# ilirlikalla/Smith-Waterman-FPGA-module

Hardware: AMD Instinct MI355X
Metric: GCUPS (higher is better)
Workload: dtype f16

## Files before the change

### smith-waterman-fpga-module_amd/csrc/swbank_bank.h

```cpp
#ifndef SWBANK_BANK_H
#define SWBANK_BANK_H

#include <dlfcn.h>
#include <hip/hip_runtime.h>
#include <rccl/rccl.h>

#include <algorithm>
#include <cmath>
#include <cstdarg>
#include <cstdio>
#include <cstdlib>
#include <cstring>
#include <atomic>
#include <condition_variable>
#include <functional>
#include <memory>
#include <mutex>
#include <numeric>
#include <thread>
#include <chrono>
#include <vector>
#if defined(__SSE2__)
#include <emmintrin.h>
#endif
// ... 341 lines not shown

 private:
  void loop(int device) {
    (void)hipSetDevice(device);
    for (;;) {
      std::function<sw_status()> f;
      {
        std::unique_lock<std::mutex> l(m_);
        cv_.wait(l, [&] { return stop_ || !q_.empty(); });
        if (q_.empty()) return;
        f = std::move(q_.front());
        q_.erase(q_.begin());
      }
      if (st_.load(std::memory_order_relaxed) == SW_OK) {
        const sw_status s = f();
        if (s != SW_OK) st_.store(s, std::memory_order_release);
      }
      done_.fetch_add(1, std::memory_order_acq_rel);
    }
  }
  std::mutex m_;
  std::condition_variable cv_;
  std::vector<std::function<sw_status()>> q_;
  bool stop_ = false;
  size_t posted_ = 0;
  std::atomic<size_t> done_{0};
  std::atomic<sw_status> st_{SW_OK};
  std::thread th_;
};

struct sw_bank {
  sw_config cfg{};
  int device = 0;
  int cus = 0;
  hipStream_t stream = nullptr;
  char err[512] = {0};

  bool have_pen = false;
  int alpha = SW_DNA_ALPHA;
  std::vector<int8_t> matrix;
  int32_t gap_open = 0, gap_extend = 0;

  bool have_query = false;
  uint64_t qid = 0;
  std::vector<uint8_t> query;
  std::vector<std::vector<uint8_t>> qset;
  bool mq_ready = false;
  DevBuf<uint32_t> mqtab, mqtab16;
  size_t mq_words = 0;
  DevBuf<uint32_t> mqpair;
  size_t mq_pair_words = 0;
  int mq_pair_segs = 0, mq_pair_rows = 0;
  uint32_t mq_pS1 = 0, mq_pS2 = 0;

  bool dirty = true;
  int R = 32, RB = 4, W = 1, col0 = 0, prof = 0;
  uint32_t S = 0, O = 0, E = 0, nv = 0, PS = 0, pad = 4;
  int32_t smax = 0;
  DevBuf<uint32_t> qtab;
  bool f16 = false;
  uint32_t nv16 = 0, PS16 = 0;
  int32_t f16_neg = 0;
  DevBuf<uint32_t> qtab16;
  DevBuf<uint32_t> qpair;
  uint32_t pair_bytes = 0, pS1 = 0, pS2 = 0;
  DevBuf<uint32_t> qpair_skew, skew_ctab;
  uint32_t skew_entries = 0;
  int32_t skew_neg = 0;
  DevBuf<uint32_t> fb_idx, fb_cnt;
  bool i32_ready = false;
  uint32_t i32_strips = 0;
  DevBuf<uint2> i32prof, i32scr;
  DevBuf<unsigned long long> best_key;
  bool al_ready = false;
  DevBuf<uint8_t> al_tab, al_res, al_hs;
  DevBuf<uint2> al_scr;
  DevBuf<uint32_t> al_dirs, al_lens, al_cig, al_list, al_hq;
  DevBuf<uint64_t> al_offs;
  DevBuf<sw_alignment> al_out;
  DevBuf<SwkAlignPlan> al_plan;
  DevBuf<unsigned long long> top_state, top_keys;
  DevBuf<int32_t> top_scores, top_hsc;
  DevBuf<uint64_t> top_hits;
  DevBuf<uint32_t> top_cnt;
  hipEvent_t ev_top = nullptr;
  SliceScratch stat_slice;
  StagedBatch stat_host;
  DevBuf<unsigned long long> stat_cnt;
  DevBuf<double> stat_par;
  std::vector<double> stat_hpar;
  hipEvent_t ev_stat = nullptr;
  SliceScratch str_slice;
  StagedBatch str_host;
  DevBuf<uint8_t> str_hstr;
  DevBuf<int32_t> str_hsc;
  hipEvent_t ev_strand = nullptr;
  SliceScratch fr_slice, fr_hits;
  StagedBatch fr_host;
  DevBuf<uint32_t> fr_lens, fr_hit_lens, fr_hit_q;
  DevBuf<uint8_t> fr_hfr;
  DevBuf<int32_t> fr_hsc;
  hipEvent_t ev_frame = nullptr;
  using Seg = qtab::Seg;
  std::vector<Seg> segs;
  qtab::Plan plan;
  DevBuf<uint2> edge[2];
// ... 330 lines not shown
```

### smith-waterman-fpga-module_amd/csrc/swbank_bank.hip

```cpp
#include "swbank_bank.h"

sw_status fail(sw_bank* b, sw_status st, const char* fmt, ...) {
  if (b) {
    va_list ap;
    va_start(ap, fmt);
    vsnprintf(b->err, sizeof(b->err), fmt, ap);
    va_end(ap);
  }
  return st;
}

extern "C" int32_t sw_device_count(void) {
  int n = 0;
  if (hipGetDeviceCount(&n) != hipSuccess) return 0;
  return n;
}

static sw_status check_device(int dev) {
  int ndev = 0;
  if (hipGetDeviceCount(&ndev) != hipSuccess || ndev <= 0) return SW_ERR_NO_DEVICE;
  if (dev < 0 || dev >= ndev) return SW_ERR_NO_DEVICE;
  hipDeviceProp_t prop;
  if (hipGetDeviceProperties(&prop, dev) != hipSuccess) return SW_ERR_NO_DEVICE;
  if (std::strncmp(prop.gcnArchName, "gfx950", 6) != 0) return SW_ERR_NO_DEVICE;
// ... 495 lines not shown
  for (const auto& u : tables) words += u.second->size();
  TableUpload up(b);
  SWOK(up.begin(words * 4));
  for (const auto& u : tables) SWOK(up.put(*u.first, *u.second));
  SWOK(up.end());
  b->plan = p;
  b->segs = t.segs;
  b->R = p.R;
  b->RB = p.RB;
  b->W = t.segs[0].W;
  b->col0 = p.col0;
  b->prof = p.prof;
  b->S = (uint32_t)p.S;
  b->O = (uint32_t)p.o;
  b->E = (uint32_t)p.e;
  b->smax = p.smax;
  b->nv = p.nv;
  b->PS = p.PS;
  b->pad = p.pad;
  b->f16 = p.f16;
  b->nv16 = p.nv16;
  b->PS16 = p.PS16;
  b->f16_neg = p.f16_neg;
  b->pair_bytes = t.pair_words * 4;
  b->pS1 = t.pS1;
  b->pS2 = t.pS2;
  b->skew_entries = (uint32_t)t.tfloor.size();
  b->skew_neg = t.skew_neg;
  b->wK = p.wK;
  b->wsegs = p.wsegs;
  b->wPS = p.prof ? (uint32_t)(64 * p.wK) : 0;
  b->wPS16 = p.prof ? (uint32_t)(128 * p.wK) : 0;
  b->wseg_words = t.wt.size() / p.wsegs;
  b->wseg_words16 = t.wt16.size() / p.wsegs;
  for (int i = 0; i < 3; ++i) {
    b->sK[i] = p.sK[i];
    b->sseg_words[i] = t.st[i].size() / (2 << i);
    b->sseg_words16[i] = t.st16[i].size() / (2 << i);
    b->sPS[i] = p.prof ? (uint32_t)(64 * p.sK[i]) : 0;
    b->sPS16[i] = p.prof ? (uint32_t)(128 * p.sK[i]) : 0;
  }
  b->i32_ready = false;
  b->al_ready = false;
  b->mq_ready = false;
  b->dirty = false;
  return SW_OK;
}

sw_status prepare_multi(sw_bank* b) {
  if (b->mq_ready) return SW_OK;
  const qtab::SetTables t =
      qtab::build_set(b->plan, b->segs, b->matrix.data(), b->qset, table_options());
  TableUpload up(b);
  SWOK(up.begin((t.t8.size() + t.t16.size() + t.tp.size()) * 4));
  SWOK(up.put(b->mqtab, t.t8));
  SWOK(up.put(b->mqtab16, t.t16));
  SWOK(up.put(b->mqpair, t.tp));
  SWOK(up.end());
  b->mq_words = t.words;
  b->mq_pair_words = t.pair_words;
  b->mq_pair_segs = t.pair_segs;
  b->mq_pair_rows = t.pair_rows;
  b->mq_pS1 = t.pS1;
  b->mq_pS2 = t.pS2;
  b->mq_ready = true;
  return SW_OK;
}

sw_status prepare_i32(sw_bank* b) {
  if (b->i32_ready) return SW_OK;
  if (b->pad + 1 > 25)
    return fail(b, SW_ERR_UNSUPPORTED, "int32 kernel: alphabet %d too large", b->alpha);
  uint32_t strips = 0;
  const std::vector<int16_t> h =
      qtab::build_i32(b->matrix.data(), b->alpha, (int)b->S, b->pad, b->query.data(),
                      (uint32_t)b->query.size(), strips);
  TableUpload up(b);
  SWOK(up.begin(h.size() * 2));
  SWOK(up.put(b->i32prof, h));
  SWOK(up.end());
  b->i32_strips = strips;
  b->i32_ready = true;
  return SW_OK;
}

extern "C" sw_status sw_bank_set_timing(sw_bank* b, int32_t enable) {
  DevGuard dev_guard(b);
  if (!b) return SW_ERR_ARG;
  if (b->is_multi()) return each_kid(b, [&](sw_bank* k) { return sw_bank_set_timing(k, enable); });
  b->timing = enable != 0;
  return SW_OK;
}

extern "C" sw_status sw_bank_timing(sw_bank* b, uint64_t* launches, double* pack_ms,
                                    double* score_ms) {
  DevGuard dev_guard(b);
  if (!b) return SW_ERR_ARG;
  double p = 0, s = 0;
  uint64_t n = 0;
  sw_status st = SW_OK;
  if (b->is_multi()) {
    for (sw_bank* k : b->kids) {
      uint64_t kn = 0;
      double kp = 0, ks = 0;
      if ((st = sw_bank_timing(k, &kn, &kp, &ks)) != SW_OK)
        return fail(b, st, "device %d: %s", k->device, k->err);
      n += kn;
      p += kp;
      s += ks;
    }
    if (launches) *launches = n;
// ... 59 lines not shown
```

### smith-waterman-fpga-module_amd/csrc/swbank_ktile.hip

```cpp
#include "swbank_kcommon.h"

namespace swk {

template <int C>
__device__ __forceinline__ void tile_chunks_local(const Lane2& t, size_t tlo, size_t thi, size_t n,
                                                  int lane, int& nch, int& nfull, int& ncl,
                                                  int tile, uint32_t ulen) {
  if (ulen) {
    const bool any = (size_t)tile * SWB_TILE < n;
    const int lx = any ? (int)ulen : 0;
    nch = max(1, (lx + C - 1) / C);
    ncl = lx == 0 ? C : lx - C * (nch - 1);
    nfull = lx / C;
    return;
  }
  uint32_t Lmax = max(t.llo, t.lhi);
  uint32_t Lmin = min(tlo < n ? t.llo : ~0u, thi < n ? t.lhi : ~0u);
  uint32_t ol = (uint32_t)lane;
  asm volatile("" : "+v"(ol));
#pragma unroll
  for (int off = 32; off >= 1; off >>= 1) {
    const int ad = (int)((ol ^ (uint32_t)off) << 2);
    Lmax = max(Lmax, (uint32_t)__builtin_amdgcn_ds_bpermute(ad, (int)Lmax));
    Lmin = min(Lmin, (uint32_t)__builtin_amdgcn_ds_bpermute(ad, (int)Lmin));
  }
  const int lx = (int)__builtin_amdgcn_readfirstlane(Lmax);
  nch = max(1, (lx + C - 1) / C);
  ncl = lx == 0 ? C : lx - C * (nch - 1);
  const uint32_t lm = __builtin_amdgcn_readfirstlane(Lmin);
  nfull = lm == ~0u ? 0 : (int)(lm / C);
}

template <int R, int RB, bool COL0, bool PROF, bool GOTOH, bool F16, bool PAIR = false,
          bool MQ = false, bool STREAM = false, int C = 8, bool BAL = false, bool TRIM = false,
          bool SKEW = false, int NB = SKEW ? (TRIM ? SWK_SKEW_ACC_TRIM : SWK_SKEW_ACC) : 1>
__global__ void __launch_bounds__(R >= 64 ? 512 : 1024) score_kernel(const ScoreArgs a) {
  static_assert(!BAL || (!MQ && !STREAM && !COL0), "balanced ranges: one query, resident batch");
  static_assert(!TRIM || (BAL && PAIR), "trimmed last chunks: the balanced pair kernel");
  static_assert(!SKEW || (PAIR && F16 && !GOTOH && !MQ && !STREAM && R == 32 && C == 8),
                "SKEW: the merged f16 pair rows, one query, resident batch");
  static_assert(!MQ || !PROF, "several queries: row-LUT or pair-table variants");
  static_assert(!STREAM || (!MQ && !PROF), "streamed batches: single-query LUT / pair variants");
  static_assert(C == 8 || (C == 4 && PAIR && !STREAM), "4-column chunks: pair tables only");
  static_assert(!PAIR || ((R == 32 || (R == 16 && GOTOH)) && F16 && !PROF && !COL0 &&
                          (!GOTOH || !MQ)),
                "PAIR: f16, merged R = 32 or Gotoh R = 16 / 32 (one query)");
  extern __shared__ __attribute__((aligned(16))) uint32_t smem[];
  const int lane = threadIdx.x & 63;
  const int wave = __builtin_amdgcn_readfirstlane(threadIdx.x >> 6);
  const int W = __builtin_amdgcn_readfirstlane(blockDim.x >> 6);
  const bool seg_in = a.edge_in != nullptr, seg_out = a.edge_out != nullptr;
  uint32_t* bestsh = smem + (PAIR ? a.PS / 4 : 0);
  constexpr int RS = SWK_RING_ROW;
  uint2* ein = reinterpret_cast<uint2*>(bestsh + W * SWB_TILE);
  uint2* ring = ein + (seg_in ? 2 * C * RS : 0);
  uint8_t* prof = reinterpret_cast<uint8_t*>(ring + (size_t)(W > 1 ? 2 * (W - 1) : 1) * C * RS);

  size_t n = a.n;
  const uint32_t* idx = a.idx;
  if (idx && a.ident && __builtin_amdgcn_readfirstlane(*a.ident)) idx = nullptr;
  const uint32_t* sidx = TRIM ? a.sidx : nullptr;
  if (TRIM && sidx && a.ident && __builtin_amdgcn_readfirstlane(*a.ident)) sidx = nullptr;
  if (idx) {
    const uint32_t cnt = __builtin_amdgcn_readfirstlane(*a.nidx);
    n = cnt > a.idx_base ? min(a.n, (size_t)(cnt - a.idx_base)) : 0;
  }
  const int ntiles = (int)((n + SWB_TILE - 1) / SWB_TILE);
  const int G = (int)gridDim.x;
  const int nunits = MQ ? ntiles * (int)a.nq : ntiles;
  int total = 0;
  uint32_t packed = a.packed;
  int* sq = reinterpret_cast<int*>(prof);
  int bs = 0, bo = 0, be = 0, bf = 0;
  if constexpr (BAL && SKEW) {
    typedef __attribute__((address_space(4))) const uint32_t plan_u32;
    plan_u32* const pp = reinterpret_cast<plan_u32*>(reinterpret_cast<uintptr_t>(a.bal_plan)) +
                         (size_t)blockIdx.x * 4;
    bs = (int)pp[0], bo = (int)pp[1];
    be = (int)pp[4], bf = (int)pp[5];
    total = (int)(pp[6] - pp[2]);
  } else if constexpr (BAL) {
    const uint4 p0 = a.bal_plan[blockIdx.x], p1 = a.bal_plan[blockIdx.x + 1];
    bs = (int)__builtin_amdgcn_readfirstlane(p0.x), bo = (int)__builtin_amdgcn_readfirstlane(p0.y);
    be = (int)__builtin_amdgcn_readfirstlane(p1.x), bf = (int)__builtin_amdgcn_readfirstlane(p1.y);
    total = (int)__builtin_amdgcn_readfirstlane(p1.z - p0.z);
  }
  const auto bal_visit = [&](int v, int& t, int& c0, int& c1) {
    const int bK = -1;
    const int bfirst = bo ? bs + 1 : bs;
    const int hh = bf > 0 ? 1 : 0;
    if (v < hh) {
      t = be, c0 = 0, c1 = bf;
    } else if (v - hh < be - bfirst) {
// ... 328 lines not shown
        }
      }
      int ntile = nunit, nqq = q;
      if constexpr (MQ) {
        if (nunit < nunits) {
          if constexpr (PAIR) {
            ntile = nunit / (int)a.nq;
          } else {
            ntile = tile + G;
            while (ntile >= ntiles) {
              ntile -= ntiles;
              ++nqq;
            }
          }
        }
      }
      if (!last) {
        load_raw<C, !MQ>(cur, c + 1, c + 1 < nfull, a.pad, packed, rlo, rhi);
      } else if (nunit < nunits) {
        if constexpr (STREAM) cur = stream_tile(ntile, packed_n);
        else
          cur = lane_targets<!MQ>(a.res, a.offs, a.lens, n, ntile, lane, packed, idx, a.ulen,
                                  a.ustride);
        if constexpr (SKEW)
          tile_chunks_local<C>(cur, (size_t)ntile * SWB_TILE + lane,
                               (size_t)ntile * SWB_TILE + lane + 64, n, lane, nch_n, nfull_n, ncl_n,
                               ntile, TRIM ? 0u : a.ulen);
        else
          tile_chunks<C>(cur, (size_t)ntile * SWB_TILE + lane,
                         (size_t)ntile * SWB_TILE + lane + 64, n, nch_n, nfull_n, ncl_n);
        if (BAL && nvend >= 0 && nvend < nch_n) ncl_n = C;
        if (BAL && nvend < 0) nvend = nch_n;
        load_raw<C, !MQ>(cur, nc0, nc0 < nfull_n, a.pad, STREAM ? packed_n : packed, rlo, rhi);
      }
      const int slot = g & 1;
      if (seg_in && wave == 0 && (last ? nunit < nunits : (MQ ? unit : tile) < nunits))
        dma_edge_chunk<C>(a.edge_in + ((size_t)(last ? nunit : MQ ? unit : tile) * a.ecols +
                                    (size_t)(last ? 0 : c + 1) * C) * 64,
                       ein + (size_t)((g + 1) & 1) * C * RS, lane);
      int rl = lane;
      if constexpr (SKEW) asm volatile("" : "+v"(rl));
      uint2* rin = wave > 0 ? ring + ((size_t)((wave - 1) * 2 + slot) * C) * RS + rl
                   : seg_in ? ein + (size_t)slot * C * RS + rl
                            : ring + 64;
      uint2* rout = wave < W - 1 ? ring + ((size_t)(wave * 2 + slot) * C) * RS + rl
                    : W > 1      ? rin
                                 : ring + rl;
      const int cu = __builtin_amdgcn_readfirstlane(c);
      uint32_t cs[SKEW ? 7 + C : 1];
      if constexpr (SKEW) {
        cst_u32* const sl = ct + (cu * C + 2);
#pragma unroll
        for (int s = 0; s < 7 + C; ++s) cs[s] = sl[s];
        if (wave == 0 && lane == 0) {
#pragma unroll
          for (int jj = 0; jj < C; ++jj) {
            if constexpr (TRIM)
              ring[jj * RS + 64] = make_uint2(cs[jj + 7], SKEW_NEG);
            else
              __atomic_store_n(reinterpret_cast<__attribute__((address_space(3))) uint32_t*>(
                                   (size_t)(lds_void_ptr)&ring[jj * RS + 64].x),
                               cs[jj + 7], __ATOMIC_RELAXED);
          }
        }
      }
      (void)cu; (void)cs;
      uint2 rv = rin[0];
      ProfLookup16<PROF && F16 ? R : 2> lkq;
      (void)lkq;
      const int ncols = TRIM && c + 1 == nch ? ncl : C;
      bool trimmed = false;
      (void)ncols;
#pragma unroll
      for (int jj = 0; jj < C; ++jj) {
        if (TRIM && jj > 0 && __builtin_expect(jj >= ncols, 0)) {
          trimmed = true;
          break;
        }
        const u16x2 upH = as_u16x2(rv.x);
        u16x2 upX = as_u16x2(rv.y);
        if (jj + 1 < C) rv = rin[(jj + 1) * RS];
        u16x2 diag = prevUpH;
        prevUpH = upH;
        const uint32_t wlo = jj < 4 ? clo.x : clo.y, whi = jj < 4 ? chi.x : chi.y;
        if constexpr (PROF && F16) {
          const auto load16 = [&](int j, ProfLookup16<R>& out) {
            const uint32_t wl = j < 4 ? clo.x : clo.y, wh = j < 4 ? chi.x : chi.y;
            const uint32_t blo = min((wl >> (8 * (j & 3))) & 0xFFu, padc);
            const uint32_t bhi = min((wh >> (8 * (j & 3))) & 0xFFu, padc);
            const uint4* plo = reinterpret_cast<const uint4*>(prof + __umul24(blo, a.PS) + 2 * pbase);
            const uint4* phi = reinterpret_cast<const uint4*>(prof + __umul24(bhi, a.PS) + 2 * pbase);
#pragma unroll
            for (int q = 0; q < R / 8; ++q) {
              const uint4 x = plo[q], y = phi[q];
              out.lo[4 * q] = x.x; out.lo[4 * q + 1] = x.y; out.lo[4 * q + 2] = x.z;
              out.lo[4 * q + 3] = x.w;
              out.hi[4 * q] = y.x; out.hi[4 * q + 1] = y.y; out.hi[4 * q + 2] = y.z;
              out.hi[4 * q + 3] = y.w;
            }
          };
          ProfLookup16<R> lk;
          if (jj == 0) load16(0, lk);
          else lk = lkq;
          if (jj + 1 < C) load16(jj + 1, lkq);
          __builtin_amdgcn_sched_barrier(0);
          if (COL0 && jj == 0 && c == 0)
            column_f16<R, RB, GOTOH, true>(lk, diag, upX, Hl, Xl, best, NOE2, NE2, NO2);
// ... 373 lines not shown
  a.ctab = tab;
  a.f16_e1 = f16_pair((int)a.E);
  a.f16_ne8 = f16_pair(-8 * (int)a.E);
}

}

#define SWK_VARIANTS(X)                                                                       \
  X(16, 4, 0, 0, 0, 0) X(16, 4, 1, 0, 0, 0) X(32, 4, 0, 0, 0, 0) X(32, 4, 1, 0, 0, 0)         \
  X(32, 8, 0, 0, 0, 0) X(64, 4, 0, 0, 0, 0) X(64, 4, 1, 0, 0, 0)                              \
  X(16, 4, 0, 0, 1, 0) X(32, 4, 0, 0, 1, 0) X(64, 4, 0, 0, 1, 0)                              \
  X(16, 4, 0, 1, 0, 0) X(16, 4, 1, 1, 0, 0) X(32, 4, 0, 1, 0, 0) X(32, 4, 1, 1, 0, 0)         \
  X(64, 4, 0, 1, 0, 0) X(64, 4, 1, 1, 0, 0)                                                   \
  X(16, 4, 0, 1, 1, 0) X(32, 4, 0, 1, 1, 0) X(64, 4, 0, 1, 1, 0)                              \
  X(16, 4, 0, 0, 0, 1) X(16, 4, 1, 0, 0, 1) X(32, 4, 0, 0, 0, 1) X(64, 4, 0, 0, 0, 1)         \
  X(16, 4, 0, 0, 1, 1)                                                                        \
  X(16, 4, 0, 1, 0, 1) X(16, 4, 1, 1, 0, 1) X(16, 4, 0, 1, 1, 1) X(32, 4, 0, 0, 1, 1)


extern "C" int swk_has_variant(int R, int RB, int col0, int prof, int gotoh, int f16) {
#define SWK_HAS(RR, BB, C0, PF, GT, FH) \
  if (R == RR && RB == BB && col0 == C0 && prof == PF && gotoh == GT && f16 == FH) return 1;
  SWK_VARIANTS(SWK_HAS)
#undef SWK_HAS
  return 0;
}

extern "C" hipError_t swk_launch_score(int R, int RB, int col0, int prof, int gotoh, int f16,
                                       const uint8_t* res, const uint64_t* offs,
                                       const uint32_t* lens, size_t n, const uint32_t* qtab,
                                       uint32_t nv, uint32_t S, uint32_t O, uint32_t E,
                                       uint32_t PS, uint32_t pad, int W, int32_t* scores,
                                       const void* edge_in, void* edge_out, uint32_t ecols,
                                       int accum, int packed, const uint32_t* idx,
                                       const uint32_t* nidx, uint32_t idx_base,
                                       const uint32_t* ident, int pair, uint32_t pS1,
                                       uint32_t pS2, uint32_t ulen, uint32_t ustride,
                                       uint32_t nq, uint32_t qwords, size_t sstride,
                                       hipStream_t st, const uint32_t* skew_tab) {
  if (n == 0) return hipSuccess;
  swk::ScoreArgs a{res,  offs, lens, n,  qtab, nv, S,
                   O,    E,    PS,   pad, scores, static_cast<const uint2*>(edge_in),
                   static_cast<uint2*>(edge_out), ecols, (uint32_t)accum, (uint32_t)packed,
                   idx, nidx, idx_base, ident, pS1, pS2,
                   swk::f16_pair(-(int)(O + E)), swk::f16_pair(-(int)E),
                   swk::f16_pair(-(int)O), nullptr, 0u, 0u, 0};
  a.ulen = ulen;
  a.ustride = ustride;
  a.nq = nq;
  a.qwords = qwords;
  a.sstride = sstride;
  const uint32_t prof_bytes = (pad + 1) * PS;
  if (nq > 1 && pair) {
    if (R == 32 && f16 && !prof && !gotoh && !col0 && (W > 4 || a.edge_in || a.edge_out))
      return swk::launch_score<32, 4, false, false, false, true, true, true, false, 4>(a, W, 0, st);
    if (R == 32 && f16 && !prof && !gotoh && !col0)
      return swk::launch_score<32, 4, false, false, false, true, true, true>(a, W, 0, st);
    return hipErrorInvalidValue;
  }
  if (nq > 1) {
#define SWK_MQ_CASE(RR, GT, FH)                                                                  \
  if (R == RR && RB == 4 && !col0 && !prof && !pair && gotoh == GT && f16 == FH)                 \
    return swk::launch_score<RR, 4, false, false, (GT != 0), (FH != 0), false, true>(a, W, 0, st);
    SWK_MQ_CASE(32, 0, 1) SWK_MQ_CASE(32, 0, 0) SWK_MQ_CASE(16, 0, 1) SWK_MQ_CASE(16, 0, 0)
    SWK_MQ_CASE(16, 1, 1) SWK_MQ_CASE(16, 1, 0) SWK_MQ_CASE(32, 1, 1) SWK_MQ_CASE(32, 1, 0)
#undef SWK_MQ_CASE
    return hipErrorInvalidValue;
  }
  if (pair) {
    if (skew_tab && (R != 32 || !f16 || prof || gotoh || col0 || edge_in || edge_out || W > 4))
      return hipErrorInvalidValue;
    if (skew_tab) {
      swk::skew_args(a, skew_tab);
      return swk::launch_score<32, 4, false, false, false, true, true, false, false, 8, false,
                               false, true>(a, W, 0, st);
    }
    if (R == 32 && f16 && !prof && !gotoh && !col0)
      return swk::launch_score<32, 4, false, false, false, true, true>(a, W, 0, st);
#define SWK_GPAIR(RR)                                                                         \
    if (R == RR && f16 && !prof && gotoh && !col0) {                                          \
      const hipError_t e = a.edge_in || a.edge_out                                            \
          ? hipErrorInvalidConfiguration                                                      \
          : swk::launch_score<RR, 4, false, false, true, true, true>(a, W, 0, st);            \
      if (e != hipErrorInvalidConfiguration) return e;                                        \
      return swk::launch_score<RR, 4, false, false, true, true, true, false, false, 4>(a, W, 0, \
                                                                                         st); \
    }
    SWK_GPAIR(32) SWK_GPAIR(16)
#undef SWK_GPAIR
    return hipErrorInvalidValue;
  }
#define SWK_CASE(RR, BB, C0, PF, GT, FH)                                                      \
  if (R == RR && RB == BB && col0 == C0 && prof == PF && gotoh == GT && f16 == FH)            \
    return swk::launch_score<RR, BB, (C0 != 0), (PF != 0), (GT != 0), (FH != 0)>(a, W,        \
                                                                               prof_bytes, st);
  SWK_VARIANTS(SWK_CASE)
#undef SWK_CASE
  return hipErrorInvalidValue;
}

#if SWK_STAMPS
extern "C" void swk_set_stamps(void* p) { swk::g_stamps_host = static_cast<uint64_t*>(p); }
#endif

namespace swk {
__global__ void __launch_bounds__(256) bal_plan_uniform(uint4* plan, uint32_t ntiles, uint32_t K,
// ... 125 lines not shown
```

### smith-waterman-fpga-module_amd/csrc/swbank_launch.hip

```cpp
#include "swbank_bank.h"

static bool one_len_bin(uint32_t min_len, uint32_t max_len) {
  if (min_len > max_len) return false;
  uint32_t shift = 0;
  while ((max_len >> shift) >= 2048u) ++shift;
  return ((max_len - min_len) >> shift) == 0;
}

void u16_gotoh_rows(const sw_bank* b, bool f16, int& R, int& W) {
  if (f16 || !b->gotoh() || b->prof || R != 32 || b->segs.size() != 1 || b->query.size() > 256)
    return;
  R = 16;
  W = std::max(1, (int)((b->query.size() + 15) / 16));
}

bool wave_preferred(const sw_bank* b, size_t n, uint32_t max_len, bool use_f16) {
  const size_t nseg = b->segs.size();
  const size_t ntiles = (n + SWB_TILE - 1) / SWB_TILE;
  const bool gotoh = b->cfg.gap_model == SW_GAP_GOTOH;
  const double tiles = (double)ntiles, W = b->segs[0].W;
  const double cu_frac = std::min(1.0, tiles / 256.0);
  const double wps = std::min(4.0, std::max(1.0, std::ceil(tiles / 256.0)) * W / 4.0);
  const bool pair_tab = use_f16 && b->pair_bytes != 0 && env_int("SWBANK_PAIR", 1) != 0;
  const double tile_base = use_f16 ? (gotoh ? (b->prof ? 7100 : pair_tab ? 8500 : 7500)
// ... 401 lines not shown

sw_status track_best_device(sw_bank* b, const int32_t* d_scores, const uint64_t* d_ids, size_t n,
                            hipStream_t st) {
  if (n > 0xFFFFFFFFull) return SW_OK;
  HIPOK(b, b->best_key.reserve(1));
  HIPOK(b, b->best_dev.reserve(3));
  HIPOK(b, swk_best_hit(d_scores, d_ids, n, b->best_key.p, b->best_dev.p, b->best_dev.p + 2, st));
  if (!b->best_ev) HIPOK(b, hipEventCreateWithFlags(&b->best_ev, hipEventDisableTiming));
  HIPOK(b, hipEventRecord(b->best_ev, st));
  b->best_kind = 2;
  return SW_OK;
}

sw_status launch_set(sw_bank* b, const uint8_t* d_res, const uint64_t* d_offs,
                     const uint32_t* d_lens, size_t n, uint32_t min_len, uint32_t max_len,
                     int32_t* d_scores, hipStream_t st, size_t sstride) {
  const size_t nq = b->qset.size();
  const uint64_t smax = (uint64_t)std::max(0, b->smax);
  const uint64_t top = std::min<uint64_t>(b->query.size(), max_len) * smax + smax;
  const bool f16_ok = b->f16 && b->f16_neg >= -2048 && env_int("SWBANK_F16", 1) != 0;
  const bool use_f16 = f16_ok && top <= 2048u;
  const bool exact = use_f16 || top <= 65535u;
  const size_t ntiles = (n + SWB_TILE - 1) / SWB_TILE;
  const char* kforce = std::getenv("SWBANK_KERNEL");
  const bool mq = env_int("SWBANK_MQ", 1) != 0 && !b->prof && !b->col0 && exact &&
                  env_int("SWBANK_I32", 0) == 0 && (b->R == 16 || b->R == 32) && b->RB == 4 &&
                  n <= 0xFFFFFFFFull &&
                  !(kforce && std::strcmp(kforce, "wave") == 0) && ntiles * nq <= 0x7FFFFFFFull;
  if (!mq) {
    const std::vector<uint8_t> longest = b->query;
    sw_status rs = SW_OK;
    for (size_t i = 0; i < nq && rs == SW_OK; ++i) {
      b->query = b->qset[i];
      b->dirty = true;
      rs = prepare(b);
      if (rs == SW_OK)
        rs = launch(b, d_res, d_offs, d_lens, n, max_len, d_scores + i * sstride, st, SWK_PACK_BYTES,
                    nullptr, nullptr, true, true, nullptr, nullptr, 0, 0, min_len);
    }
    b->query = longest;
    b->dirty = true;
    const size_t L = strlen(b->last_kernel);
    snprintf(b->last_kernel + L, sizeof(b->last_kernel) - L, " x%zu queries", nq);
    return rs;
  }
  sw_status rs = prepare_multi(b);
  if (rs != SW_OK) return rs;
  const bool gotoh = b->gotoh();
  const int prow = std::max(b->mq_pair_rows, 32);
  const size_t slots = (prow > 256 ? 1 : prow > 128 ? 2 : 4) * (size_t)std::max(b->cus, 1);
  const bool mpair = b->mq_pair_segs > 0 && use_f16 && nq <= slots &&
                     8 * (slots - slots / nq * nq) <= slots;
  const size_t nseg = mpair ? (size_t)b->mq_pair_segs : b->segs.size();
  snprintf(b->last_kernel, sizeof(b->last_kernel), "tile %s%s R=%d W=%d segs=%zu queries=%zu",
           use_f16 ? "f16" : "u16", mpair ? " pair" : "", b->R,
           mpair ? std::min(prow / 32, (int)(b->query.size() + 31) / 32) : b->segs[0].W, nseg,
           nq);
  HIPOK(b, hipStreamWaitEvent(st, b->ev_ready, 0));
  HIPOK(b, hipStreamWaitEvent(st, b->ev_used, 0));
  sw_bank::Ev ev{};
  if (b->timing) {
    HIPOK(b, hipEventCreate(&ev.a));
    HIPOK(b, hipEventCreate(&ev.c));
    HIPOK(b, hipEventRecord(ev.a, st));
    ev.b = ev.a;
  }
  const uint32_t ecols = (max_len + 7) / 8 * 8;
  const uint32_t *perm = nullptr, *perm_n = nullptr, *ident = nullptr;
  if (ntiles > 1 && !one_len_bin(min_len, max_len) && env_int("SWBANK_DSORT", 1) != 0) {
    HIPOK(b, b->dperm.reserve(n + 2));
    const size_t sw = swk_sort_scratch_bytes() / 4;
    if (b->dsort.cap < sw) {
      HIPOK(b, b->dsort.reserve(sw));
      HIPOK(b, hipMemsetAsync(b->dsort.p, 0, sw * 4, st));
    }
    HIPOK(b, swk_sort_lens(d_lens, n, max_len, b->dperm.p, b->dperm.p + n, b->dperm.p + n + 1,
                           b->dsort.p, st));
    ++b->ctr.device_sorts;
    perm = b->dperm.p;
    perm_n = b->dperm.p + n;
    ident = b->dperm.p + n + 1;
  }
  size_t span = n;
  if (nseg > 1) {
    const size_t budget = (size_t)std::max(1, env_int("SWBANK_EDGE_MB", 2048)) << 20;
    const size_t per_tile = (size_t)ecols * 64 * sizeof(uint2) * nq;
    span = std::min(n, std::max<size_t>(1, budget / per_tile) * SWB_TILE);
    const size_t words = (span + SWB_TILE - 1) / SWB_TILE * ecols * 64 * nq;
    HIPOK(b, b->edge[0].reserve(words));
    HIPOK(b, b->edge[1].reserve(words));
  }
  const uint32_t* tabs = use_f16 ? b->mqtab16.p : b->mqtab.p;
  for (size_t p0 = 0; p0 < n; p0 += span) {
    const size_t np = std::min(span, n - p0);
    const uint64_t* offs = perm ? d_offs : d_offs + p0;
    const uint32_t* lens = perm ? d_lens : d_lens + p0;
    int32_t* scores = perm ? d_scores : d_scores + p0;
    for (size_t sg = 0; sg < nseg; ++sg) {
      const void* ein = sg > 0 ? b->edge[(sg - 1) & 1].p : nullptr;
      void* eout = sg + 1 < nseg ? b->edge[sg & 1].p : nullptr;
      if (mpair) {
        const int rows = std::min(prow, (int)b->query.size() - (int)sg * prow);
        const int Wp = std::max(1, (rows + 31) / 32);
        HIPOK(b, swk_launch_score(32, 4, 0, 0, 0, 1, d_res, offs, lens, np,
                                  b->mqpair.p + sg * nq * b->mq_pair_words, b->nv16, b->S, b->O,
                                  b->E, (uint32_t)b->mq_pair_words * 4, b->pad, Wp, scores, ein,
                                  eout, ecols, sg > 0 ? 1 : 0, (int)SWK_PACK_BYTES,
                                  perm ? perm + p0 : nullptr, perm_n, (uint32_t)p0, ident, 1,
                                  b->mq_pS1, b->mq_pS2, 0, 0, (uint32_t)nq,
                                  (uint32_t)b->mq_pair_words, sstride, st));
        continue;
      }
      HIPOK(b, swk_launch_score(b->R, b->RB, 0, 0, gotoh ? 1 : 0, use_f16 ? 1 : 0, d_res, offs,
                                lens, np, tabs + b->segs[sg].off, use_f16 ? b->nv16 : b->nv,
                                b->S, b->O, b->E, 0, b->pad, b->segs[sg].W, scores, ein, eout,
                                ecols, sg > 0 ? 1 : 0, (int)SWK_PACK_BYTES,
                                perm ? perm + p0 : nullptr, perm_n, (uint32_t)p0, ident, 0, 0, 0,
                                0, 0, (uint32_t)nq, (uint32_t)b->mq_words, sstride, st));
    }
  }
  HIPOK(b, hipEventRecord(b->ev_used, st));
  if (b->timing) {
    HIPOK(b, hipEventRecord(ev.c, st));
    b->events.push_back(ev);
  }
  return SW_OK;
}

extern "C" sw_status sw_score_batch_device(sw_bank* b, const uint8_t* d_res,
                                           const uint64_t* d_offs, const uint32_t* d_lens,
                                           const uint64_t* d_ids, size_t n, uint32_t max_len,
                                           int32_t* d_scores, void* stream) {
  DevGuard dev_guard(b);
  return sw_score_batch_device_range(b, d_res, d_offs, d_lens, d_ids, n, 0, max_len, d_scores,
                                     stream);
}

extern "C" sw_status sw_score_batch_device_range(sw_bank* b, const uint8_t* d_res,
                                                 const uint64_t* d_offs, const uint32_t* d_lens,
                                                 const uint64_t* d_ids, size_t n,
                                                 uint32_t min_len, uint32_t max_len,
                                                 int32_t* d_scores, void* stream) {
  DevGuard dev_guard(b);
  if (!b) return SW_ERR_ARG;
  if (min_len > max_len) return fail(b, SW_ERR_ARG, "min_len %u > max_len %u", min_len, max_len);
  b->best_kind = 0;
  b->best_root = false;
  if (const sw_status fs = take_fault(b, 0); fs != SW_OK) return fs;
  if (n == 0) return SW_OK;
  if (!d_res || !d_offs || !d_lens || !d_scores) return fail(b, SW_ERR_ARG, "null device buffer");
  if (b->is_multi()) {
    if (b->qset.size() > 1 && d_ids) return fail(b, SW_ERR_UNSUPPORTED, "best hit over a query set");
    return multi_device(b, d_res, d_offs, d_lens, d_ids, n, min_len, max_len, d_scores,
                        reinterpret_cast<hipStream_t>(stream), false);
  }
  sw_status st = prepare(b);
  if (st != SW_OK) return st;
  HIPOK(b, hipSetDevice(b->device));
  hipStream_t hs = stream ? reinterpret_cast<hipStream_t>(stream) : b->stream;
  if (b->qset.size() > 1) {
    if (d_ids) return fail(b, SW_ERR_UNSUPPORTED, "best hit over a query set");
    return launch_set(b, d_res, d_offs, d_lens, n, min_len, max_len, d_scores, hs, n);
  }
// ... 42 lines not shown
```

### smith-waterman-fpga-module_amd/csrc/swbank_qtab.h

```cpp
#ifndef SWBANK_QTAB_H
#define SWBANK_QTAB_H

#include <algorithm>
#include <cstdint>
#include <cstdio>
#include <cstring>
#include <vector>

#include "swbank.h"

namespace qtab {

inline uint16_t f16_score_bits(int v) {
  return __builtin_bit_cast(uint16_t, (_Float16)((float)v * (1.0f / 2048.0f)));
}

enum class Entry { U8, F16Hi, F16 };
inline size_t entry_bytes(Entry k) { return k == Entry::F16 ? 2 : 1; }
inline uint32_t entry_pad(Entry k) { return k == Entry::U8 ? 0xFFu : k == Entry::F16Hi ? 0xBCu : 0xBC00u; }
inline uint32_t entry_of(Entry k, int S, int s) {
  return k == Entry::U8 ? (uint32_t)(uint8_t)(S - s)
                        : k == Entry::F16Hi ? (uint32_t)(f16_score_bits(s) >> 8) : f16_score_bits(s);
}

// ... 114 lines not shown
      qp[(size_t)c * stride + i] = (T)entry_of(k, S, m[q[r0 + i] * A + c]);
  std::memcpy(out, qp.data(), qp.size() * sizeof(T));
}
inline void profile(Entry k, const uint8_t* q, int qlen, int r0, int nrows, const int8_t* m, int A,
                    int S, size_t stride, uint32_t* out) {
  if (k == Entry::F16)
    profile_as<uint16_t>(k, q, qlen, r0, nrows, m, A, S, stride, out);
  else
    profile_as<uint8_t>(k, q, qlen, r0, nrows, m, A, S, stride, out);
}

inline size_t append_rows(const Plan& p, Entry k, const uint8_t* q, int qlen, int r0, int nrows,
                          size_t stride, const int8_t* m, std::vector<uint32_t>& t) {
  const size_t base = t.size();
  t.resize(base + (p.prof ? (size_t)(p.A + 1) * stride * entry_bytes(k) / 4 : (size_t)nrows));
  if (p.prof)
    profile(k, q, qlen, r0, nrows, m, p.A, p.S, stride, t.data() + base);
  else
    row_words(k, q, qlen, r0, nrows, m, p.A, p.S, t.data() + base);
  return base;
}

inline void pair_strides(uint32_t NR, uint32_t& pS1, uint32_t& pS2) {
  const uint32_t B = 4 * NR;
  pS2 = (B + 15) / 16 * 16;
  while ((pS2 / 16) % 16 != 1) pS2 += 16;
  pS1 = (4 * pS2 + B + 15) / 16 * 16;
  while ((pS1 / 16) % 16 != 4) pS1 += 16;
}

inline std::vector<uint32_t> pair_table(const uint8_t* q, int qlen, int r0, uint32_t NR,
                                        const int8_t* m, int A, uint32_t pS1, uint32_t pS2,
                                        int add = 0, int pad = -2048, int add0 = 0) {
  const uint32_t bytes = 16 + 4 * pS1 + 4 * pS2 + 4 * NR;
  const uint32_t padw = (uint32_t)f16_score_bits(pad + add) * 0x10001u;
  std::vector<uint32_t> t(bytes / 4, padw);
  auto word = [&](int r, int x, int y) -> uint32_t {
    const int ad = add + (r % 8 == 0 ? add0 : 0);
    if (r0 + r >= qlen) return (uint32_t)f16_score_bits(pad + ad) * 0x10001u;
    const int c = q[r0 + r];
    return (uint32_t)f16_score_bits(m[c * A + x] + ad) |
           (uint32_t)f16_score_bits(m[c * A + y] + ad) << 16;
  };
  for (int x = 0; x < A; ++x)
    for (int y = 0; y < A; ++y) {
      const uint32_t base = (16 + x * pS1 + y * pS2) / 4;
      for (uint32_t k = 0; k + 1 < NR; ++k) t[base + k] = word((int)k + 1, x, y);
    }
  for (int x = 0; x < A; ++x)
    for (int y = 0; y < A; ++y) t[(16 + x * pS1 + y * pS2) / 4 - 1] = word(0, x, y);
  return t;
}

struct QueryTables {
  std::vector<Seg> segs;
  std::vector<uint32_t> tab, tab16;
  std::vector<uint32_t> tpair;
  uint32_t pS1 = 0, pS2 = 0, pair_words = 0;
  std::vector<uint32_t> tskew, tfloor;
  int32_t skew_neg = 0;
  std::vector<uint32_t> wt, wt16, st[3], st16[3];
};

inline QueryTables build_query(const Plan& p, const int8_t* m, const uint8_t* q) {
  QueryTables t;
  const int A = p.A, R = p.R, qlen = p.qlen;
  const Entry k16 = p.prof ? Entry::F16 : Entry::F16Hi;
  for (int r0 = 0; r0 < std::max(qlen, 1); r0 += p.seg_rows) {
    const int rows = std::min(p.seg_rows, std::max(qlen, 1) - r0);
    const int W = std::max(1, (rows + R - 1) / R);
    Seg sg{W, 0, 0};
    sg.off = append_rows(p, Entry::U8, q, qlen, r0, W * R, p.PS, m, t.tab);
    if (p.f16) sg.off16 = append_rows(p, k16, q, qlen, r0, W * R, p.PS16 / 2, m, t.tab16);
    t.segs.push_back(sg);
  }
  if (p.f16 && !p.prof && !p.col0 && A == SW_DNA_ALPHA &&
      (p.gotoh ? R == 16 || R == 32 : R == 32 && t.segs.size() == 1 && t.segs[0].W <= 4)) {
    const uint32_t NR = (uint32_t)t.segs[0].W * R;
    pair_strides(NR, t.pS1, t.pS2);
    for (size_t sg = 0; sg < t.segs.size(); ++sg) {
      const std::vector<uint32_t> one =
          pair_table(q, qlen, (int)sg * p.seg_rows, NR, m, A, t.pS1, t.pS2);
      t.pair_words = (uint32_t)one.size();
      t.tpair.insert(t.tpair.end(), one.begin(), one.end());
    }
  }
  if (!t.tpair.empty() && !p.gotoh && 2 * p.e <= 2048) {
    const int e = p.e, spad = -std::min(2048 - 2 * e, p.S * std::max(qlen, 1));
    t.tskew = pair_table(q, qlen, 0, (uint32_t)t.segs[0].W * R, m, A, t.pS1, t.pS2, 2 * e, spad,
                         -8 * e);
    t.tfloor.resize(2048 + 32);
    for (size_t k = 0; k < t.tfloor.size(); ++k)
      t.tfloor[k] = (uint32_t)f16_score_bits(std::min(2048, e * ((int)k - 3))) * 0x10001u;
    t.skew_neg = 5 * e + std::min(p.smin, spad) + 2 * e - 8 * e - p.o;
  }
  auto wave_tables = [&](int wrows, int nsegs, std::vector<uint32_t>& wt,
                         std::vector<uint32_t>& wt16) {
    for (int sg = 0; sg < nsegs; ++sg) {
      append_rows(p, Entry::U8, q, qlen, sg * wrows, wrows, wrows, m, wt);
      if (p.f16) append_rows(p, k16, q, qlen, sg * wrows, wrows, wrows, m, wt16);
    }
  };
  wave_tables(64 * p.wK, p.wsegs, t.wt, t.wt16);
  for (int i = 0; i < 3; ++i)
    if (p.sK[i]) wave_tables(64 * p.sK[i], 2 << i, t.st[i], t.st16[i]);
  return t;
}

struct SetTables {
  size_t words = 0;
  std::vector<uint32_t> t8, t16;
  std::vector<uint32_t> tp;
  size_t pair_words = 0;
  int pair_segs = 0, pair_rows = 0;
  uint32_t pS1 = 0, pS2 = 0;
};

inline SetTables build_set(const Plan& p, const std::vector<Seg>& segs, const int8_t* m,
                           const std::vector<std::vector<uint8_t>>& qset, const Options& opt) {
  SetTables t;
  const int R = p.R, seg_rows = segs[0].W * R;
  t.words = segs.back().off + (size_t)segs.back().W * R;
  t.t8.resize(qset.size() * t.words);
  if (p.f16) t.t16.resize(qset.size() * t.words);
  for (size_t i = 0; i < qset.size(); ++i)
    for (size_t sg = 0; sg < segs.size(); ++sg) {
      const size_t base = i * t.words + segs[sg].off;
      const int r0 = (int)sg * seg_rows, nr = segs[sg].W * R, ql = (int)qset[i].size();
      row_words(Entry::U8, qset[i].data(), ql, r0, nr, m, p.A, p.S, t.t8.data() + base);
      if (p.f16)
        row_words(Entry::F16Hi, qset[i].data(), ql, r0, nr, m, p.A, p.S, t.t16.data() + base);
    }
  if (p.f16 && !p.prof && !p.gotoh && !p.col0 && p.A == SW_DNA_ALPHA && opt.mq_pair != 0) {
    const uint32_t NR = opt.mq_pair_rows == 128 ? 128 : opt.mq_pair_rows == 256 ? 256 : 512;
    t.pair_rows = (int)NR;
    pair_strides(NR, t.pS1, t.pS2);
    t.pair_segs = std::max(1, (p.qlen + (int)NR - 1) / (int)NR);
    for (int sg = 0; sg < t.pair_segs; ++sg)
      for (const std::vector<uint8_t>& qi : qset) {
        const std::vector<uint32_t> one =
            pair_table(qi.data(), (int)qi.size(), sg * (int)NR, NR, m, p.A, t.pS1, t.pS2);
        t.pair_words = one.size();
        t.tp.insert(t.tp.end(), one.begin(), one.end());
      }
  }
  return t;
}

inline std::vector<int16_t> build_i32(const int8_t* m, int A, int S, uint32_t pad, const uint8_t* q,
                                      uint32_t qlen, uint32_t& strips) {
  strips = std::max(1u, (qlen + 255) / 256);
  std::vector<int16_t> h((size_t)strips * (pad + 1) * 64 * 4, 0);
  for (uint32_t s = 0; s < strips; ++s)
    for (uint32_t c = 0; c <= pad; ++c)
      for (uint32_t l = 0; l < 64; ++l)
        for (uint32_t k = 0; k < 4; ++k) {
          const uint32_t r = s * 256 + 4 * l + k;
          int v = 0;
          if (r < qlen) v = c < (uint32_t)A ? m[q[r] * A + c] : S - 255;
          h[(((size_t)s * (pad + 1) + c) * 64 + l) * 4 + k] = (int16_t)v;
        }
  return h;
}

inline std::vector<uint8_t> build_align(const std::vector<int8_t>& matrix,
                                        const std::vector<uint8_t>* queries, size_t nq) {
  size_t ql = 0;
  for (size_t i = 0; i < nq; ++i) ql += queries[i].size();
  std::vector<uint8_t> t(nq * 8 + matrix.size() + ql);
  uint8_t* codes = t.data() + nq * 8 + matrix.size();
  size_t at = 0;
  for (size_t i = 0; i < nq; ++i) {
    const uint32_t e[2] = {(uint32_t)at, (uint32_t)queries[i].size()};
    std::memcpy(t.data() + i * 8, e, 8);
    if (!queries[i].empty()) std::memcpy(codes + at, queries[i].data(), queries[i].size());
    at += queries[i].size();
  }
  if (!matrix.empty()) std::memcpy(t.data() + nq * 8, matrix.data(), matrix.size());
  return t;
}

}

#endif
```

Measured before the change: 14810.

## Extend skewed f16 pair kernel to multi-query segmented pair path

Builds skewed pair tables and a floor table for query sets and uploads them to the device. The multi-query pair launch switches to a SKEW kernel variant with four-column chunks and four accumulators when the score range fits in f16. This is meant to bring the cheaper skewed recurrence, already used for single queries, to multi-segment query sets. It adds extra table memory and host build time, and widens the static_assert, which risks correctness at segment edges.

```diff
diff --git a/smith-waterman-fpga-module_amd/csrc/swbank_bank.h b/smith-waterman-fpga-module_amd/csrc/swbank_bank.h
--- a/smith-waterman-fpga-module_amd/csrc/swbank_bank.h
+++ b/smith-waterman-fpga-module_amd/csrc/swbank_bank.h
@@ -417,6 +417,9 @@
   size_t mq_pair_words = 0;
   int mq_pair_segs = 0, mq_pair_rows = 0;
   uint32_t mq_pS1 = 0, mq_pS2 = 0;
+  DevBuf<uint32_t> mqpair_skew, mq_skew_ctab;
+  uint32_t mq_skew_entries = 0;
+  int32_t mq_skew_neg = 0;
 
   bool dirty = true;
   int R = 32, RB = 4, W = 1, col0 = 0, prof = 0;
diff --git a/smith-waterman-fpga-module_amd/csrc/swbank_bank.hip b/smith-waterman-fpga-module_amd/csrc/swbank_bank.hip
--- a/smith-waterman-fpga-module_amd/csrc/swbank_bank.hip
+++ b/smith-waterman-fpga-module_amd/csrc/swbank_bank.hip
@@ -571,11 +571,16 @@
   const qtab::SetTables t =
       qtab::build_set(b->plan, b->segs, b->matrix.data(), b->qset, table_options());
   TableUpload up(b);
-  SWOK(up.begin((t.t8.size() + t.t16.size() + t.tp.size()) * 4));
+  SWOK(up.begin(
+      (t.t8.size() + t.t16.size() + t.tp.size() + t.tps.size() + t.tfloor.size()) * 4));
   SWOK(up.put(b->mqtab, t.t8));
   SWOK(up.put(b->mqtab16, t.t16));
   SWOK(up.put(b->mqpair, t.tp));
+  SWOK(up.put(b->mqpair_skew, t.tps));
+  SWOK(up.put(b->mq_skew_ctab, t.tfloor));
   SWOK(up.end());
+  b->mq_skew_entries = t.tps.empty() ? 0u : (uint32_t)t.tfloor.size();
+  b->mq_skew_neg = t.skew_neg;
   b->mq_words = t.words;
   b->mq_pair_words = t.pair_words;
   b->mq_pair_segs = t.pair_segs;
diff --git a/smith-waterman-fpga-module_amd/csrc/swbank_ktile.hip b/smith-waterman-fpga-module_amd/csrc/swbank_ktile.hip
--- a/smith-waterman-fpga-module_amd/csrc/swbank_ktile.hip
+++ b/smith-waterman-fpga-module_amd/csrc/swbank_ktile.hip
@@ -33,12 +33,15 @@
 
 template <int R, int RB, bool COL0, bool PROF, bool GOTOH, bool F16, bool PAIR = false,
           bool MQ = false, bool STREAM = false, int C = 8, bool BAL = false, bool TRIM = false,
-          bool SKEW = false, int NB = SKEW ? (TRIM ? SWK_SKEW_ACC_TRIM : SWK_SKEW_ACC) : 1>
+          bool SKEW = false,
+          int NB = SKEW ? (TRIM || C == 4 ? SWK_SKEW_ACC_TRIM : SWK_SKEW_ACC) : 1>
 __global__ void __launch_bounds__(R >= 64 ? 512 : 1024) score_kernel(const ScoreArgs a) {
   static_assert(!BAL || (!MQ && !STREAM && !COL0), "balanced ranges: one query, resident batch");
   static_assert(!TRIM || (BAL && PAIR), "trimmed last chunks: the balanced pair kernel");
-  static_assert(!SKEW || (PAIR && F16 && !GOTOH && !MQ && !STREAM && R == 32 && C == 8),
-                "SKEW: the merged f16 pair rows, one query, resident batch");
+  static_assert(!SKEW || (PAIR && F16 && !GOTOH && !STREAM && R == 32 &&
+                          (C == 8 ? !MQ : NB == SWK_SKEW_ACC_TRIM && !BAL)),
+                "SKEW: the merged f16 pair rows, resident batch; one query, or 4-column chunks "
+                "(query sets and segments) with four accumulators");
   static_assert(!MQ || !PROF, "several queries: row-LUT or pair-table variants");
   static_assert(!STREAM || (!MQ && !PROF), "streamed batches: single-query LUT / pair variants");
   static_assert(C == 8 || (C == 4 && PAIR && !STREAM), "4-column chunks: pair tables only");
@@ -473,7 +476,7 @@
         cst_u32* const sl = ct + (cu * C + 2);
 #pragma unroll
         for (int s = 0; s < 7 + C; ++s) cs[s] = sl[s];
-        if (wave == 0 && lane == 0) {
+        if (wave == 0 && lane == 0 && (C == 8 || !seg_in)) {
 #pragma unroll
           for (int jj = 0; jj < C; ++jj) {
             if constexpr (TRIM)
@@ -953,6 +956,12 @@
   a.sstride = sstride;
   const uint32_t prof_bytes = (pad + 1) * PS;
   if (nq > 1 && pair) {
+    if (skew_tab && (R != 32 || !f16 || prof || gotoh || col0)) return hipErrorInvalidValue;
+    if (skew_tab) {
+      swk::skew_args(a, skew_tab);
+      return swk::launch_score<32, 4, false, false, false, true, true, true, false, 4, false,
+                               false, true>(a, W, 0, st);
+    }
     if (R == 32 && f16 && !prof && !gotoh && !col0 && (W > 4 || a.edge_in || a.edge_out))
       return swk::launch_score<32, 4, false, false, false, true, true, true, false, 4>(a, W, 0, st);
     if (R == 32 && f16 && !prof && !gotoh && !col0)
diff --git a/smith-waterman-fpga-module_amd/csrc/swbank_launch.hip b/smith-waterman-fpga-module_amd/csrc/swbank_launch.hip
--- a/smith-waterman-fpga-module_amd/csrc/swbank_launch.hip
+++ b/smith-waterman-fpga-module_amd/csrc/swbank_launch.hip
@@ -477,10 +477,15 @@
   const bool mpair = b->mq_pair_segs > 0 && use_f16 && nq <= slots &&
                      8 * (slots - slots / nq * nq) <= slots;
   const size_t nseg = mpair ? (size_t)b->mq_pair_segs : b->segs.size();
-  snprintf(b->last_kernel, sizeof(b->last_kernel), "tile %s%s R=%d W=%d segs=%zu queries=%zu",
+  const uint64_t skew_cols = ((uint64_t)max_len + 7) / 8 * 8;
+  const bool skew = mpair && nseg > 1 && b->mq_skew_entries != 0 &&
+                    top + (uint64_t)b->E * ((uint64_t)prow + skew_cols) <= 2048u &&
+                    b->mq_skew_neg >= -2048 && skew_cols + 16 <= b->mq_skew_entries &&
+                    env_int("SWBANK_SKEW", 1) != 0;
+  snprintf(b->last_kernel, sizeof(b->last_kernel), "tile %s%s R=%d W=%d segs=%zu queries=%zu%s",
            use_f16 ? "f16" : "u16", mpair ? " pair" : "", b->R,
            mpair ? std::min(prow / 32, (int)(b->query.size() + 31) / 32) : b->segs[0].W, nseg,
-           nq);
+           nq, skew ? " skew" : "");
   HIPOK(b, hipStreamWaitEvent(st, b->ev_ready, 0));
   HIPOK(b, hipStreamWaitEvent(st, b->ev_used, 0));
   sw_bank::Ev ev{};
@@ -528,12 +533,15 @@
         const int rows = std::min(prow, (int)b->query.size() - (int)sg * prow);
         const int Wp = std::max(1, (rows + 31) / 32);
         HIPOK(b, swk_launch_score(32, 4, 0, 0, 0, 1, d_res, offs, lens, np,
-                                  b->mqpair.p + sg * nq * b->mq_pair_words, b->nv16, b->S, b->O,
+                                  (skew ? b->mqpair_skew.p : b->mqpair.p) +
+                                      sg * nq * b->mq_pair_words,
+                                  b->nv16, b->S, b->O,
                                   b->E, (uint32_t)b->mq_pair_words * 4, b->pad, Wp, scores, ein,
                                   eout, ecols, sg > 0 ? 1 : 0, (int)SWK_PACK_BYTES,
                                   perm ? perm + p0 : nullptr, perm_n, (uint32_t)p0, ident, 1,
                                   b->mq_pS1, b->mq_pS2, 0, 0, (uint32_t)nq,
-                                  (uint32_t)b->mq_pair_words, sstride, st));
+                                  (uint32_t)b->mq_pair_words, sstride, st,
+                                  skew ? b->mq_skew_ctab.p : nullptr));
         continue;
       }
       HIPOK(b, swk_launch_score(b->R, b->RB, 0, 0, gotoh ? 1 : 0, use_f16 ? 1 : 0, d_res, offs,
diff --git a/smith-waterman-fpga-module_amd/csrc/swbank_qtab.h b/smith-waterman-fpga-module_amd/csrc/swbank_qtab.h
--- a/smith-waterman-fpga-module_amd/csrc/swbank_qtab.h
+++ b/smith-waterman-fpga-module_amd/csrc/swbank_qtab.h
@@ -190,6 +190,19 @@
   return t;
 }
 
+inline int skew_pad(const Plan& p, int qlen) {
+  return -std::min(2048 - 2 * p.e, p.S * std::max(qlen, 1));
+}
+inline std::vector<uint32_t> floor_table(int e) {
+  std::vector<uint32_t> f(2048 + 32);
+  for (size_t k = 0; k < f.size(); ++k)
+    f[k] = (uint32_t)f16_score_bits(std::min(2048, e * ((int)k - 3))) * 0x10001u;
+  return f;
+}
+inline int32_t skew_lowest(const Plan& p, int spad) {
+  return 5 * p.e + std::min(p.smin, spad) + 2 * p.e - 8 * p.e - p.o;
+}
+
 struct QueryTables {
   std::vector<Seg> segs;
   std::vector<uint32_t> tab, tab16;
@@ -224,13 +237,11 @@
     }
   }
   if (!t.tpair.empty() && !p.gotoh && 2 * p.e <= 2048) {
-    const int e = p.e, spad = -std::min(2048 - 2 * e, p.S * std::max(qlen, 1));
+    const int e = p.e, spad = skew_pad(p, qlen);
     t.tskew = pair_table(q, qlen, 0, (uint32_t)t.segs[0].W * R, m, A, t.pS1, t.pS2, 2 * e, spad,
                          -8 * e);
-    t.tfloor.resize(2048 + 32);
-    for (size_t k = 0; k < t.tfloor.size(); ++k)
-      t.tfloor[k] = (uint32_t)f16_score_bits(std::min(2048, e * ((int)k - 3))) * 0x10001u;
-    t.skew_neg = 5 * e + std::min(p.smin, spad) + 2 * e - 8 * e - p.o;
+    t.tfloor = floor_table(e);
+    t.skew_neg = skew_lowest(p, spad);
   }
   auto wave_tables = [&](int wrows, int nsegs, std::vector<uint32_t>& wt,
                          std::vector<uint32_t>& wt16) {
@@ -252,6 +263,8 @@
   size_t pair_words = 0;
   int pair_segs = 0, pair_rows = 0;
   uint32_t pS1 = 0, pS2 = 0;
+  std::vector<uint32_t> tps, tfloor;
+  int32_t skew_neg = 0;
 };
 
 inline SetTables build_set(const Plan& p, const std::vector<Seg>& segs, const int8_t* m,
@@ -281,6 +294,17 @@
         t.pair_words = one.size();
         t.tp.insert(t.tp.end(), one.begin(), one.end());
       }
+    if (2 * p.e <= 2048) {
+      const int e = p.e, spad = std::min(p.smin, 0);
+      for (int sg = 0; sg < t.pair_segs; ++sg)
+        for (const std::vector<uint8_t>& qi : qset) {
+          const std::vector<uint32_t> one = pair_table(qi.data(), (int)qi.size(), sg * (int)NR, NR,
+                                                       m, p.A, t.pS1, t.pS2, 2 * e, spad, -8 * e);
+          t.tps.insert(t.tps.end(), one.begin(), one.end());
+        }
+      t.skew_neg = skew_lowest(p, spad);
+      t.tfloor = floor_table(e);
+    }
   }
   return t;
 }
```

Measured after the change: 14780. About the same (-0.2%).
